# felicityin/zkvm-brainfuck

Hardware: AMD Instinct MI355X
Metric: core-proof wall-time (ms) + NTT HBM GB/s, fibonacci trace 2^22 rows (lower is better)
Workload: dtype u32 (KoalaBear mod-p); 1 GPU; fibo_x4 stdin[255]: 3,767,729 cycles, Cpu trace 2^22 rows, full core proof (84 FRI queries, 16 PoW bits); cycles=3767729, parallelism=replicas x1

## Files before the change

### zkvm-brainfuck_amd/csrc/gpu.h

```cpp
#pragma once
#include <hip/hip_runtime.h>

#include <cstdint>
#include <cstdio>
#include <cstdlib>
#include <functional>
#include <initializer_list>
#include <atomic>
#include <chrono>
#include <map>
#include <mutex>
#include <unordered_map>
#include <unordered_set>
#include <stdexcept>
#include <string>
#include <vector>

#include "kb.h"

namespace bfz {

struct HipError : std::runtime_error {
  using std::runtime_error::runtime_error;
};
// ... 38 lines not shown
      return p;
    }
    if (carve) {
      if (slab_left_ < bytes) {
        if (slab_left_ >= GRAIN) {
          size_of_[slab_next_] = slab_left_;
          free_[slab_left_].push_back(slab_next_);
        }
        slab_next_ = (uint8_t*)device_malloc(SLAB);
        slab_left_ = SLAB;
      }
      void* p = slab_next_;
      slab_next_ += bytes;
      slab_left_ -= bytes;
      size_of_[p] = bytes;
      return p;
    }
    void* p = device_malloc(bytes);
    size_of_[p] = bytes;
    own_.insert(p);
    return p;
  }
  uint64_t mallocs() const { return mallocs_; }
  double malloc_ms() const { return malloc_ns_ * 1e-6; }
  size_t bytes() {
    std::lock_guard<std::mutex> lk(mu_);
    return held_;
  }
  void release(void* p) {
    if (!p) return;
    std::lock_guard<std::mutex> lk(mu_);
    auto it = size_of_.find(p);
    if (it == size_of_.end()) return;
    free_[it->second].push_back(p);
  }
  void trim() {
    std::lock_guard<std::mutex> lk(mu_);
    for (auto kv = free_.begin(); kv != free_.end();) {
      auto& v = kv->second;
      for (size_t i = 0; i < v.size();) {
        if (!own_.count(v[i])) {
          i++;
          continue;
        }
        (void)hipFree(v[i]);
        held_ -= kv->first;
        size_of_.erase(v[i]);
        own_.erase(v[i]);
        v[i] = v.back();
        v.pop_back();
      }
      kv = v.empty() ? free_.erase(kv) : std::next(kv);
    }
  }
  ~DevicePool() {}

 private:
  static bool slabs_on() {
    static const bool on = [] {
      const char* e = std::getenv("BFZ_POOL_SLABS");
      return !(e && e[0] == '0' && !e[1]);
    }();
    return on;
  }
  void* device_malloc(size_t bytes) {
    void* p = nullptr;
    const auto t0 = std::chrono::steady_clock::now();
    HIP_CHECK(hipMalloc(&p, bytes));
    malloc_ns_ += (uint64_t)std::chrono::duration_cast<std::chrono::nanoseconds>(
                      std::chrono::steady_clock::now() - t0).count();
    mallocs_++;
    held_ += bytes;
    return p;
  }
  std::map<size_t, std::vector<void*>> free_;
  std::unordered_map<void*, size_t> size_of_;
  std::unordered_set<void*> own_;
  uint8_t* slab_next_ = nullptr;
  size_t slab_left_ = 0;
  size_t held_ = 0;
  std::atomic<uint64_t> mallocs_{0}, malloc_ns_{0};
  std::mutex mu_;
};

void preload_register(const void* kernel);
struct PreloadKernels {
  PreloadKernels(std::initializer_list<const void*> ks) {
    for (const void* k : ks) preload_register(k);
  }
};
double preload_kernels();

constexpr int MAX_LANES = 4;
constexpr int DEFAULT_INFLIGHT = 2;
struct Lane {
  int id = 0;
  hipStream_t stream = nullptr;
  DevicePool pool;
  uint8_t* stage = nullptr;
  size_t stage_cap = 0, stage_off = 0;
  uint8_t* box = nullptr;
  size_t box_cap = 0;
  hipEvent_t spin = nullptr;
  static constexpr int NGEV = 4;
  hipEvent_t gev[NGEV] = {};
  void* gbox = nullptr;
  size_t gcap = 0;
  uint32_t* tbox = nullptr;
  size_t tcap = 0;
};
Lane& lane();
Lane* lane_at(int i);
size_t lane_pool_bytes(int i);
struct LaneScope {
  Lane* prev;
  explicit LaneScope(Lane* l);
  ~LaneScope();
};

void run_lanes(int n, const std::function<void(int)>& body);

DevicePool& pool();
DevicePool& resident_pool();
struct ResidentScope {
  DevicePool* prev;
  ResidentScope();
  ~ResidentScope();
};

template <class T>
struct DBuf {
  T* p = nullptr;
  size_t n = 0;
  bool owned = true;
  DevicePool* from = nullptr;
  DBuf() = default;
  explicit DBuf(size_t count) { reset(count); }
  DBuf(const DBuf&) = delete;
  DBuf& operator=(const DBuf&) = delete;
  DBuf(DBuf&& o) noexcept : p(o.p), n(o.n), owned(o.owned), from(o.from) { o.p = nullptr; o.n = 0; }
  DBuf& operator=(DBuf&& o) noexcept {
    if (this != &o) { free(); p = o.p; n = o.n; owned = o.owned; from = o.from; o.p = nullptr; o.n = 0; }
    return *this;
  }
  static DBuf borrow(T* ptr, size_t count) {
    DBuf b;
// ... 135 lines not shown
```

### zkvm-brainfuck_amd/csrc/prover.h

```cpp
#pragma once
#include <array>
#include <memory>
#include <string>
#include <vector>

#include "gpu.h"
#include "machine.h"
#include "merkle.h"

namespace bfz {

using kb::EF;

struct Challenger {
  uint32_t st[16] = {0};
  uint32_t in[8] = {0};
  int nin = 0;
  uint32_t out[8] = {0};
  int nout = 0;
  void duplex();
  void observe(uint32_t v);
  void observe_digest(const uint32_t d[8]);
  void observe_ef(const EF& e);
  uint32_t sample();
// ... 50 lines not shown
  double reduce_kernel_ms = 0, reduce_kernel_bytes = 0;
  int reduce_kernel_launches = 0;
  double perm_rows = 0, perm_idft = 0, perm_dft = 0, perm_hash = 0;
  double main_idft = 0, main_dft = 0, main_hash = 0;
  double main_cells = 0, perm_cells = 0;
  double spin = 0;
};

std::unique_ptr<ProvingKey> setup(const std::string& program_src);

void commit_lde(CMat& cm, const uint32_t* evals, size_t n, int w, uint32_t domain_shift,
                hipStream_t st);

struct ProveOptions {
  int num_queries = 84;
  bool timing = false;
  bool observe_openings = true;
  bool fault_device_challenger = false;
};

std::vector<uint8_t> prove(const ProvingKey& pk, const uint8_t* stdin_data, size_t nin,
                           const ProveOptions& opt, StageTimes* times,
                           std::vector<uint8_t>* output_stream = nullptr,
                           uint64_t* cycles = nullptr);

struct DeviceTraces {
  std::vector<int> chips;
  std::vector<DBuf<uint32_t>> evals;
  std::vector<size_t> heights;
};
void upload_host_traces(const int* chips, const uint32_t* const* mats, const size_t* heights,
                        const size_t* widths, size_t n, DeviceTraces& dt, hipStream_t st);
std::vector<uint8_t> prove_device(const ProvingKey& pk, DeviceTraces& dt, const ProveOptions& opt,
                                  StageTimes* times);

void host_mark(const char* what);
std::vector<uint8_t> acquire_proof_buffer();
void release_proof_buffer(std::vector<uint8_t>&& v);

struct MainData {
  DeviceTraces dt;
  std::vector<int> order;
  std::vector<int> chip;
  std::vector<size_t> hn;
  Round mainr;
  bool root_on_host = true;
};
void commit_main(MainData& md);
Challenger challenger_after_pk(const ProvingKey& pk);
std::vector<uint8_t> open_main(const ProvingKey& pk, MainData& md, const Challenger& ch,
                               const ProveOptions& opt, Challenger* after = nullptr);

int num_queries_from_env();
bool observe_openings_from_env();

}
```

### zkvm-brainfuck_amd/csrc/prover.hip

```cpp
#include "prover.h"
#include "pipeline.h"

#include <algorithm>
#include <cerrno>
#include <chrono>
#include <cstdio>
#include <cstdlib>
#include <cstring>
#include <mutex>

#include "fri.h"
#include "host_p2.h"
#include "logup.h"
#include "ntt.h"
#include "poseidon2.h"
#include "quotient.h"
#include "tracegen.h"
#include "verifier.h"

namespace bfz {

using namespace kb;

static constexpr int LOG_BLOWUP = 1;
// ... 325 lines not shown
  if (timed) tm->end(bs, st, split->dft);
  if (tm && tm->on) {
    tm->end(b, st, &times->lde_ms);
    times->lde_bytes += 12.0 * (double)n * w;
    times->lde_elem_stages += 3.0 * (double)n * cm.log_n * w;
    times->lde_calls++;
  }
}

void commit_lde(CMat& cm, const uint32_t* evals, size_t n, int w, uint32_t domain_shift,
                hipStream_t st) {
  lde_into(cm, evals, n, w, domain_shift, st, nullptr, nullptr);
}

static Mailbox* roots_boxes() {
  static Mailbox boxes[MAX_LANES];
  return boxes;
}

static void warm_lane_host() {
  lane_host_reserve();
  Lane& ln = lane();
  roots_boxes()[ln.id].reserve(4096);
  for (int g = 0; g < Lane::NGEV; g++)
    if (!ln.gev[g]) HIP_CHECK(hipEventCreateWithFlags(&ln.gev[g], hipEventDisableTiming));
  if (!ln.gbox) {
    ln.gcap = 4096;
    HIP_CHECK(hipHostMalloc(&ln.gbox, ln.gcap * sizeof(EF), hipHostMallocDefault));
  }
  if (!ln.tbox) {
    ln.tcap = (size_t)1 << 18;
    HIP_CHECK(hipHostMalloc(reinterpret_cast<void**>(&ln.tbox), ln.tcap * 4, hipHostMallocDefault));
  }
}

std::unique_ptr<ProvingKey> setup(const std::string& src) {
  ResidentScope rs;
  warm_lane_host();
  twiddles().ensure(TWIDDLE_LOG_MAX);
  auto pk = std::make_unique<ProvingKey>();
  pk->program = Program::parse(src);
  hipStream_t st = stream();
  int chips[2] = {CHIP_PROGRAM, CHIP_BYTE};
  std::vector<uint32_t> t[2];
  size_t h[2];
  for (int i = 0; i < 2; i++) h[i] = prep_trace(chips[i], pk->program, t[i]);
  int ord[2] = {0, 1};
  if (h[1] > h[0] || (h[1] == h[0] && std::strcmp(CHIP_INFO[chips[1]].name, CHIP_INFO[chips[0]].name) < 0))
    std::swap(ord[0], ord[1]);
  pk->idx_of_chip.fill(-1);
  pk->prep.mats.resize(2);
  pk->prep_evals.resize(2);
  for (int k = 0; k < 2; k++) {
    const int i = ord[k];
    const int w = CHIP_INFO[chips[i]].prep_w;
    pk->chip_of[k] = chips[i];
    pk->idx_of_chip[chips[i]] = k;
    DBuf<uint32_t> rm(h[i] * w);
    HIP_CHECK(hipMemcpyAsync(rm.p, t[i].data(), t[i].size() * 4, hipMemcpyHostToDevice, st));
    pk->prep_evals[k].reset(h[i] * w);
    transpose_bitrev(rm.p, h[i], w, pk->prep_evals[k].p, st);
    HIP_CHECK(hipStreamSynchronize(st));
    lde_into(pk->prep.mats[k], pk->prep_evals[k].p, h[i], w, ONE, st, nullptr, nullptr);
  }
  pk->prep.commit(st);
  return pk;
// ... 1 lines not shown

void upload_host_traces(const int* chips, const uint32_t* const* mats, const size_t* heights,
                        const size_t* widths, size_t n, DeviceTraces& dt, hipStream_t st) {
  dt.chips.clear();
  dt.evals.clear();
  dt.heights.clear();
  bool seen[NUM_CHIPS] = {};
  for (size_t i = 0; i < n; i++) {
    const int c = chips[i];
    if (c < 0 || c >= NUM_CHIPS || seen[c]) throw std::runtime_error("traces: bad or repeated chip id");
    seen[c] = true;
    const size_t h = heights[i];
    const int w = CHIP_INFO[c].main_w;
    if ((size_t)w != widths[i])
      throw std::runtime_error(std::string("traces: width mismatch for ") + CHIP_INFO[c].name);
    if (h < 1 || (h & (h - 1)) || h > ((size_t)1 << 23))
      throw std::runtime_error(std::string("traces: height not a power of two in [1, 2^23] for ") +
                               CHIP_INFO[c].name);
    DBuf<uint32_t> rm(h * w);
    upload_bulk(rm.p, mats[i], h * w * 4, st);
    if (count_noncanonical(rm.p, h * w, st))
      throw std::runtime_error(std::string("traces: non-canonical field word (>= p) in ") +
                               CHIP_INFO[c].name);
    DBuf<uint32_t> ev(h * w);
    transpose_bitrev(rm.p, h, w, ev.p, st);
    dt.chips.push_back(c);
    dt.evals.push_back(std::move(ev));
    dt.heights.push_back(h);
  }
  if (!seen[0]) throw std::runtime_error("traces: the Cpu chip is required");
}

namespace {
struct ProofScope {
  EvTimer ev;
  StageTimes local;
  StageTimes* tms;
  hipEvent_t e_total = nullptr;
  ProofScope(bool timing, StageTimes* times) : tms(times ? times : &local) {
    ev.on = timing && times;
    if (!ev.on) {
      for (KernelProbe* p : {&ntt_probe(), &p2_probe(), &open_probe(), &reduce_probe()})
        if (p->on) p->on = false;
      return;
    }
    ntt_probe().reset();
    ntt_probe().on = true;
    p2_probe().reset();
    p2_probe().on = true;
    open_probe().reset();
    open_probe().on = true;
    reduce_probe().reset();
    reduce_probe().on = true;
    e_total = ev.begin(stream());
  }
  void finish() {
    if (!ev.on) return;
    ev.end(e_total, stream(), &tms->total);
    ev.collect();
    tms->quotient -= tms->spin;
    tms->total -= tms->spin;
    KernelProbe& pr = ntt_probe();
    pr.collect();
    pr.on = false;
    tms->ntt_kernel_ms = pr.ms;
    tms->ntt_kernel_bytes = pr.bytes;
    tms->ntt_kernel_launches = pr.launches;
    KernelProbe& p2 = p2_probe();
    p2.collect();
    p2.on = false;
    tms->p2_kernel_ms = p2.ms;
    tms->p2_perms = p2.bytes;
    tms->p2_launches = p2.launches;
    KernelProbe& op = open_probe();
    op.collect();
    op.on = false;
    tms->open_kernel_ms = op.ms;
    tms->open_kernel_bytes = op.bytes;
    tms->open_kernel_launches = op.launches;
    KernelProbe& rp = reduce_probe();
    rp.collect();
    rp.on = false;
    tms->reduce_kernel_ms = rp.ms;
    tms->reduce_kernel_bytes = rp.bytes;
    tms->reduce_kernel_launches = rp.launches;
  }
  ~ProofScope() {
    (void)hipStreamSynchronize(stream());
    staging_reset();
    if (ev.on)
      for (KernelProbe* p : {&ntt_probe(), &p2_probe(), &open_probe(), &reduce_probe()}) p->on = false;
  }
};

void commit_main_impl(MainData& md, ProofScope& ps, bool fetch_root = true) {
  hipStream_t st = stream();
  DeviceTraces& dt = md.dt;
  const int nc = (int)dt.chips.size();
  md.order.resize(nc);
  for (int i = 0; i < nc; i++) md.order[i] = i;
  std::sort(md.order.begin(), md.order.end(), [&](int a, int b) {
    if (dt.heights[a] != dt.heights[b]) return dt.heights[a] > dt.heights[b];
    return std::strcmp(CHIP_INFO[dt.chips[a]].name, CHIP_INFO[dt.chips[b]].name) < 0;
  });
  md.chip.resize(nc);
  md.hn.resize(nc);
  for (int k = 0; k < nc; k++) {
    md.chip[k] = dt.chips[md.order[k]];
    md.hn[k] = dt.heights[md.order[k]];
  }
  htrace().mark("main commit");
  hipEvent_t e0 = ps.ev.on ? ps.ev.begin(st) : nullptr;
  Span span("commit to main traces");
  const Plan plan = make_plan();
  md.mainr = Round();
  md.mainr.mats.resize(nc);
  LdeSplit split{ps.tms ? &ps.tms->main_idft : nullptr, ps.tms ? &ps.tms->main_dft : nullptr};
  for (int k = 0; k < nc; k++) {
    lde_into(md.mainr.mats[k], dt.evals[md.order[k]].p, md.hn[k], CHIP_INFO[md.chip[k]].main_w, ONE,
             st, &ps.ev, ps.tms, &plan, &chip_next_cols(md.chip[k]).main, ps.tms ? &split : nullptr);
    if (ps.tms) ps.tms->main_cells += (double)md.hn[k] * CHIP_INFO[md.chip[k]].main_w;
  }
  hipEvent_t eh = ps.ev.on ? ps.ev.begin(st) : nullptr;
  htrace().mark("main LDE queued");
  md.mainr.commit(st, fetch_root);
  htrace().mark("main tree queued");
  if (ps.ev.on) ps.ev.end(eh, st, &ps.tms->main_hash);
  md.root_on_host = fetch_root;
  if (ps.ev.on) ps.ev.end(e0, st, &ps.tms->main_commit);
}

std::vector<uint8_t> open_impl(const ProvingKey& pk, MainData& md, Challenger ch,
                               const ProveOptions& opt, ProofScope& ps, Challenger* after = nullptr);

struct QuotXchg {
  std::vector<int> chips;
  std::vector<size_t> off;
  size_t total = 0;
  DBuf<uint32_t> send, recv;
  hipEvent_t ready = nullptr;
  QuotXchg() = default;
  QuotXchg(const QuotXchg&) = delete;
  QuotXchg& operator=(const QuotXchg&) = delete;
  ~QuotXchg() {
    if (ready) (void)hipEventDestroy(ready);
  }
};
static uint32_t* quot_part(std::vector<DBuf<uint32_t>>& qv, const std::vector<size_t>& hn,
                           const Plan& plan, int k, int rank) {
  const size_t n = hn[k], b = plan.blk(2 * n), t0 = (size_t)rank * b;
  return qv[k].p + (t0 / n) * 4 * n + (t0 % n);
}
static void quot_pack(QuotXchg& x, std::vector<DBuf<uint32_t>>& qv, const std::vector<size_t>& hn,
                      const Plan& plan, hipStream_t st) {
  x.off.assign(x.chips.size(), 0);
// ... 35 lines not shown
  for (int j = 0; j < plan.G; j++)
    for (size_t i = 0; i < x.chips.size(); i++)
      if (j != plan.k) {
        const int k = x.chips[i];
        const size_t n = hn[k], b = plan.blk(2 * n);
        cp.push_back({x.recv.p + (size_t)j * x.total + x.off[i], quot_part(qv, hn, plan, k, j), b,
                      n, b, 4});
      }
  copy2d_batch(cp, st);
  x.send.free();
}
}

void commit_main(MainData& md) {
  ProofScope ps(false, nullptr);
  commit_main_impl(md, ps);
  HIP_CHECK(hipStreamSynchronize(stream()));
}

std::vector<uint8_t> open_main(const ProvingKey& pk, MainData& md, const Challenger& ch,
                               const ProveOptions& opt, Challenger* after) {
  ProofScope ps(false, nullptr);
  return open_impl(pk, md, ch, opt, ps, after);
}

Challenger challenger_after_pk(const ProvingKey& pk) {
  Challenger ch;
  ch.observe_digest(pk.prep.tree.root);
  for (int i = 0; i < 7; i++) ch.observe(0);
  return ch;
}

std::vector<uint8_t> prove_device(const ProvingKey& pk, DeviceTraces& dt, const ProveOptions& opt,
                                  StageTimes* times) {
  ProofScope ps(opt.timing, times);
  MainData md;
  md.dt = std::move(dt);
  commit_main_impl(md, ps, false);
  auto proof = open_impl(pk, md, challenger_after_pk(pk), opt, ps);
  htrace().mark("open returned");
  ps.finish();
  dt = std::move(md.dt);
  return proof;
}

namespace {
std::vector<uint8_t> open_impl(const ProvingKey& pk, MainData& md, Challenger ch,
                               const ProveOptions& opt, ProofScope& ps, Challenger* after) {
  hipStream_t st = stream();
  EvTimer& ev = ps.ev;
  StageTimes* tms = ps.tms;
  DeviceTraces& dt = md.dt;
  const std::vector<int>& order = md.order;
  const std::vector<int>& chip = md.chip;
  const std::vector<size_t>& hn = md.hn;
  Round& mainr = md.mainr;
  const int nc = (int)chip.size();
  const Plan plan = make_plan();
  const ShardCtx* shard = shard_ctx();

  htrace().mark("open start");
  DBuf<DevChallenger> dc_d(1);
  {
    DevChallenger dc;
    std::memcpy(dc.st, ch.st, sizeof(dc.st));
    std::memcpy(dc.in, ch.in, sizeof(dc.in));
    std::memcpy(dc.out, ch.out, sizeof(dc.out));
    dc.nin = ch.nin;
    dc.nout = ch.nout;
    if (opt.fault_device_challenger)
      dc.st[15] = dc.st[15] ? dc.st[15] - 1 : 1;
// ... 544 lines not shown
      if (e != hipErrorNotReady) HIP_CHECK(e);
    }
    const size_t b0 = g ? gend[g - 1] : 0, b1 = std::max(gend[g], b0);
    std::copy(gbox + b0, gbox + b1, opened.begin() + b0);
  };
  if (grouped) {
    int have = -1;
    for (int r = 0; r < 4; r++) {
      while (have < group_of(r)) wait_group(++have);
      if (opt.observe_openings)
        for (size_t i = 0; i < rounds[r]->mats.size(); i++)
          for (int j = 0; j < mp[r][i].npts; j++)
            for (int c = 0; c < rounds[r]->mats[i].lde.width; c++)
              ch.observe_ef(opened[mp[r][i].off[j] + c]);
    }
    while (have < NGROUP - 1) wait_group(++have);
    htrace().mark("opened observed");
  } else if (opt.observe_openings) {
    htrace().mark("opened summed");
    for (int r = 0; r < 4; r++)
      for (size_t i = 0; i < rounds[r]->mats.size(); i++)
        for (int j = 0; j < mp[r][i].npts; j++)
          for (int c = 0; c < rounds[r]->mats[i].lde.width; c++)
            ch.observe_ef(opened[mp[r][i].off[j] + c]);
  }
  const EF fri_alpha = ch.sample_ef();
  htrace().mark("fri alpha");

  DBuf<EF> alpha_yab(1 + 2 * std::max<size_t>(red_jobs.size(), 1));
  upload_async(alpha_yab.p, &fri_alpha, sizeof(EF), st);
  reduce_prep(red_cols_d.p, col_prep_d.p, red_mats_d.p, mat_prep_d.p, job_prep_d.p,
              (int)red_jobs.size(), opened_dev, alpha_yab.p, alpha_yab.p + 1, st);
  std::map<int, DBuf<EF>> ro;
  for (size_t ji = 0; ji < red_jobs.size(); ji++) {
    const RedJob& j = red_jobs[ji];
    const size_t H = (size_t)1 << j.lh;
    const bool sh = plan.sharded(H);
    const size_t t0 = sh ? plan.row0(H) : 0, cnt = sh ? plan.blk(H) : H;
    DBuf<EF> r(cnt);
    const Invd& d = invd.at(j.lh);
    reduce_range(red_cols_d.p + j.col0, red_mats_d.p + j.mat0, j.nmats, H, t0, cnt, d.pa(),
                 j.has_b ? d.pb() : nullptr, alpha_yab.p + 1 + 2 * ji, j.has_b, r.p - t0, st,
                 (int)j.ncols);
    ro.emplace(j.lh, std::move(r));
  }
  if (ev.on) ev.end(e3, st, &tms->open);

  hipEvent_t e4 = ev.on ? ev.begin(st) : nullptr;
  struct FriLayer {
    DBuf<EF> v;
    size_t e0 = 0;
    bool local = false;
  };
  std::vector<FriLayer> layers;
  std::vector<MerkleTree> trees;
  {
    const size_t H = (size_t)1 << Lmax;
    layers.push_back({std::move(ro.at(Lmax)), plan.sharded(H) ? plan.row0(H) : 0, plan.sharded(H)});
  }
  ro.erase(Lmax);
  if (ch.nin != 0) throw std::runtime_error("FRI: unexpected pending challenger input");
  DBuf<uint32_t> dstate(16);
  upload_async(dstate.p, ch.st, 64, st);
  const int nrounds = Lmax - LOG_BLOWUP;
  DBuf<EF> betas(std::max(nrounds, 1));
  size_t len = (size_t)1 << Lmax;
  static const size_t FRI_SHARD_MIN = [] {
    const char* e = std::getenv("BFZ_FRI_SHARD_MIN");
    return e ? (size_t)std::strtoull(e, nullptr, 10) : (size_t)1 << 18;
  }();
  auto fri_sharded = [&](size_t h) { return plan.sharded(h) && h >= FRI_SHARD_MIN; };
  auto gather = [&](DBuf<EF>& v, size_t len) {
    DBuf<EF> all(len);
    coll_sync(st);
    shard->allgather(v.p, plan.blk(len) * sizeof(EF), all.p);
    v = std::move(all);
  };
// ... 17 lines not shown
      flush_fold();
      FriTailRounds a;
      a.logh0 = log2i(h);
      a.nr = log2i(len) - LOG_BLOWUP;
      a.in = cur.v.p;
      a.state = dstate.p;
      a.beta = betas.p + rd;
      size_t nw = 0, nv = 0;
      for (int r = 0; r < a.nr; r++) {
        nw += 8 * ((h >> r) * 2 - 1);
        nv += h >> r;
      }
      tail_trees.reset(nw);
      tail_layers.reset(nv);
      nw = nv = 0;
      for (int r = 0; r < a.nr; r++) {
        const size_t hr = h >> r;
        const EF* rows = r ? tail_layers.p + nv - 2 * hr : cur.v.p;
        trees.emplace_back();
        MerkleTree& t = trees.back();
        t.mats = {MatRef{(const uint32_t*)rows, hr, 8}};
        t.layers.resize(log2i(hr) + 1);
        a.tree[r] = tail_trees.p + nw;
        for (size_t L = 0; L < t.layers.size(); L++) {
          t.layers[L] = DBuf<uint32_t>::borrow(tail_trees.p + nw, 8 * (hr >> L));
          nw += 8 * (hr >> L);
        }
        a.layer[r] = tail_layers.p + nv;
        const int lgh = log2i(hr);
        a.add[r] = ro.count(lgh) ? ro.at(lgh).p : nullptr;
        layers.push_back({DBuf<EF>::borrow(tail_layers.p + nv, hr), 0, false});
        nv += hr;
      }
      fri_tail_rounds(a, st);
      len = h >> (a.nr - 1);
      break;
    }
    if (cur.local && !fri_sharded(h)) {
      gather(cur.v, len);
      cur.e0 = 0;
      cur.local = false;
    }
    const bool loc = cur.local;
    const size_t i0 = loc ? plan.row0(h) : 0, cnt = loc ? plan.blk(h) : h;
    trees.emplace_back();
    MerkleTree& t = trees.back();
    std::function<void(size_t, size_t, uint32_t*)> fused;
    if (pend.in) {
      const PendingFold pf = pend;
      EF* out = cur.v.p;
      fused = [pf, out, h, &st](size_t, size_t, uint32_t* dig) {
        fri_fold_leaves(pf.in, out, h, pf.beta, pf.add, dig, st);
      };
      pend = PendingFold{};
    }
    merkle_from_rows8(t, (const uint32_t*)(cur.v.p - 2 * i0), h, st, false,
                      RootChallenge{dstate.p, betas.p + rd}, loc, fused);
    DBuf<EF> next(cnt);
    const int lgh = log2i(h);
    if (!loc && ro.count(lgh) && plan.sharded(h)) gather(ro.at(lgh), h);
    const EF* add = ro.count(lgh) ? ro.at(lgh).p : nullptr;
    if (!loc && h / 2 >= FRI_FUSE_MIN) pend = PendingFold{cur.v.p, betas.p + rd, add, h};
    else fri_fold_range(cur.v.p, next.p, h, i0, cnt, betas.p + rd, add, st);
    layers.push_back({std::move(next), i0, loc});
    len = h;
  }
  flush_fold();
  const int nt = (int)trees.size();
  if (nt > MAX_FRI_ROUNDS) throw std::runtime_error("FRI: too many rounds");
  const int nq = opt.num_queries;

  auto owner_shift = [](const MerkleTree& t, int L) {
    const int nl = (int)t.layers.size() - 1;
    return L < t.sharded_below ? nl - L - t.shard_log : -1;
  };
  std::vector<GatherSeg> segs;
  const int ncommit = nt;
  auto lit = [&](uint32_t v) { segs.push_back({nullptr, 0, 0, v, 0, 1, -1, 0}); };
  lit(4);
  for (int r = 0; r < 4; r++) {
    const Round& R = *rounds[r];
    const int lrm = (int)R.tree.layers.size() - 1;
    lit((uint32_t)R.mats.size());
    for (const CMat& m : R.mats) {
      const int lh = log2i(m.lde.height);
      lit((uint32_t)m.lde.width);
      segs.push_back({m.rows(), (uint64_t)m.stride(), (uint32_t)(Lmax - lh), 0, 1,
                      (uint32_t)m.lde.width, m.sharded ? lh - plan.lg : -1, 0});
    }
    lit((uint32_t)lrm);
    for (int L = 0; L < lrm; L++)
      segs.push_back({R.tree.layers[L].p, 1, (uint32_t)(Lmax - lrm + L), 1, 8, 8,
                      owner_shift(R.tree, L), 0});
  }
  lit((uint32_t)ncommit);
  for (int i = 0; i < ncommit; i++) {
    const FriLayer& fl = layers[i];
    segs.push_back({(const uint32_t*)(fl.v.p - fl.e0), 1, (uint32_t)i, 1, 4, 4,
                    fl.local ? Lmax - i - plan.lg : -1, 0});
    const int lm = (int)trees[i].layers.size() - 1;
// ... 112 lines not shown
    write_vals(mp[2][k].off[1], pw);
    w.u32(2);
    write_vals(mp[3][2 * k].off[0], 4);
    write_vals(mp[3][2 * k + 1].off[0], 4);
    w.ef(cums[k]);
  }
  w.u32((uint32_t)ncommit);
  for (int i = 0; i < ncommit; i++) w.digest(trees[i].root);
  w.u32((uint32_t)nq);
  w.raw(words, nwords);
  w.ef(fin[0]);
  w.u32(witness);
  htrace().mark("serialized");
  return w.take();
}
}

std::vector<uint8_t> prove_events(const ProvingKey& pk, const DeviceEvents& ev,
                                  const ProveOptions& opt, StageTimes* times) {
  hipStream_t st = stream();
  const bool timing = opt.timing && times;
  hipEvent_t a = nullptr, b = nullptr;
  if (timing) {
    HIP_CHECK(hipEventCreate(&a));
    HIP_CHECK(hipEventCreate(&b));
    HIP_CHECK(hipEventRecord(a, st));
  }
  htrace().mark("proof start", true);
  static const bool pool_diag = std::getenv("BFZ_HOST_TRACE") != nullptr;
  const uint64_t m0 = lane().pool.mallocs();
  const double t0 = lane().pool.malloc_ms();
  Span span("prove_shard");
  DeviceTraces dt;
  {
    Span gen("generate traces for shard");
    generate_traces_device(ev, dt, st);
  }
  htrace().mark("traces launched");
  if (timing) HIP_CHECK(hipEventRecord(b, st));
  auto proof = prove_device(pk, dt, opt, times);
  htrace().mark("proof returned");
  if (pool_diag)
    std::fprintf(stderr, "pool: %llu hipMalloc in this proof, %.3f ms of host time\n",
                 (unsigned long long)(lane().pool.mallocs() - m0), lane().pool.malloc_ms() - t0);
  if (timing) {
    float ms = 0;
    HIP_CHECK(hipEventElapsedTime(&ms, a, b));
    times->trace = ms;
    times->total += ms;
    HIP_CHECK(hipEventDestroy(a));
    HIP_CHECK(hipEventDestroy(b));
  }
  return proof;
}

std::vector<uint8_t> prove(const ProvingKey& pk, const uint8_t* in, size_t nin,
                           const ProveOptions& opt, StageTimes* times,
                           std::vector<uint8_t>* output_stream, uint64_t* cycles) {
  HostEvents& h = scratch_events();
  execute_into(pk.program, in, nin, h);
  DeviceEvents ev;
  upload_events(h, pk.program, ev, stream());
  if (output_stream) *output_stream = h.output;
  if (cycles) *cycles = h.global_clk;
  return prove_events(pk, ev, opt, times);
}

static PreloadKernels preload_prover{(const void*)&k_pack_fri_tail};

}
```

### zkvm-brainfuck_amd/csrc/runtime.hip

```cpp
#include <dlfcn.h>

#include "gpu.h"

#include <algorithm>
#include <condition_variable>
#include <cstring>
#include <mutex>
#include <thread>
#include <vector>

namespace bfz {

namespace {
std::mutex g_lanes_mu;
Lane* g_lanes[MAX_LANES] = {};
thread_local Lane* tl_lane = nullptr;
Lane* make_lane(int id) {
  auto* l = new Lane();
  l->id = id;
  HIP_CHECK(hipStreamCreateWithFlags(&l->stream, hipStreamNonBlocking));
  return l;
}
}

Lane* lane_at(int i) {
  if (i < 0 || i >= MAX_LANES) throw std::runtime_error("lane index out of range");
  std::lock_guard<std::mutex> lk(g_lanes_mu);
  if (!g_lanes[i]) g_lanes[i] = make_lane(i);
  return g_lanes[i];
}
size_t lane_pool_bytes(int i) {
  if (i < 0 || i >= MAX_LANES) throw std::runtime_error("lane index out of range");
  Lane* l;
  {
    std::lock_guard<std::mutex> lk(g_lanes_mu);
    l = g_lanes[i];
  }
  return l ? l->pool.bytes() : 0;
}
Lane& lane() {
  if (tl_lane) return *tl_lane;
  static Lane* d = lane_at(0);
  return *d;
}
LaneScope::LaneScope(Lane* l) : prev(tl_lane) { tl_lane = l; }
LaneScope::~LaneScope() { tl_lane = prev; }

namespace {
thread_local DevicePool* tl_pool = nullptr;
}
DevicePool& pool() { return tl_pool ? *tl_pool : lane().pool; }
DevicePool& resident_pool() {
  static DevicePool* p = new DevicePool();
// ... 13 lines not shown
  std::call_once(once, [&] {
    const char* e = std::getenv("BFZ_PRELOAD");
    if (e && e[0] == '0' && !e[1]) return;
    const auto t0 = std::chrono::steady_clock::now();
    for (const void* k : preload_list()) {
      hipFuncAttributes a;
      HIP_CHECK(hipFuncGetAttributes(&a, k));
    }
    ms = std::chrono::duration<double, std::milli>(std::chrono::steady_clock::now() - t0).count();
  });
  return ms;
}

void run_lanes(int n, const std::function<void(int)>& body) {
  std::exception_ptr err;
  std::mutex mu;
  auto one = [&](int i) {
    try {
      ApiLockScope held;
      LaneScope ls(lane_at(i));
      body(i);
      HIP_CHECK(hipStreamSynchronize(stream()));
    } catch (...) {
      std::lock_guard<std::mutex> lk(mu);
      if (!err) err = std::current_exception();
    }
  };
  std::vector<std::thread> th;
  for (int i = 1; i < n; i++) th.emplace_back(one, i);
  one(0);
  for (auto& t : th) t.join();
  if (err) std::rethrow_exception(err);
}
hipStream_t stream() { return lane().stream; }

void quiesce() noexcept {
  for (Lane* l : g_lanes)
    if (l && l->stream) (void)hipStreamSynchronize(l->stream);
}

namespace {
struct Roctx {
  int (*push)(const char*) = nullptr;
  int (*pop)() = nullptr;
  Roctx() {
    void* h = dlopen("librocprofiler-sdk-roctx.so", RTLD_NOW | RTLD_LOCAL);
    if (!h) h = dlopen("/opt/rocm/lib/librocprofiler-sdk-roctx.so", RTLD_NOW | RTLD_LOCAL);
    if (!h) return;
    push = reinterpret_cast<int (*)(const char*)>(dlsym(h, "roctxRangePushA"));
    pop = reinterpret_cast<int (*)()>(dlsym(h, "roctxRangePop"));
    if (!push || !pop) push = nullptr, pop = nullptr;
  }
};
const Roctx& roctx() {
  static const Roctx r;
  return r;
}
}
void roctx_push(const char* name) noexcept {
  if (roctx().push) roctx().push(name);
}
void roctx_pop() noexcept {
  if (roctx().pop) roctx().pop();
}

KernelProbe& ntt_probe() {
  static KernelProbe* k = new KernelProbe();
  return *k;
}

KernelProbe& p2_probe() {
// ... 333 lines not shown
```

### zkvm-brainfuck_amd/csrc/tracegen.h

```cpp
#pragma once
#include "gpu.h"
#include "machine.h"
#include "prover.h"

namespace bfz {

struct DeviceEvents {
  DBuf<CpuEvent> cpu;
  DBuf<AluEvent> alu;
  DBuf<JumpEvent> jump;
  DBuf<MemInstrEvent> meminstr;
  DBuf<IoEvent> io;
  DBuf<MemoryEvent> memory;
  DBuf<Instruction> prog;
  size_t n[NUM_CHIPS] = {};
  size_t height[NUM_CHIPS] = {};
  bool included[NUM_CHIPS] = {};
  uint64_t global_clk = 0;
};

void upload_events(const ExecutionRecord& rec, DeviceEvents& ev, hipStream_t st);

void upload_events(const HostEvents& h, const Program& prog, DeviceEvents& ev, hipStream_t st);
void set_event_meta(DeviceEvents& ev, const EventCounts& n, uint64_t global_clk);
size_t count_invalid_events(const DeviceEvents& ev, hipStream_t st);
void expand_cycles(const Cycle* d, size_t n, DeviceEvents& ev, EventCounts& n_out, size_t* invalid,
                   hipStream_t st);
void* pinned_alloc(size_t bytes);
void pinned_free(void* p);

void generate_traces_device(const DeviceEvents& ev, DeviceTraces& dt, hipStream_t st);

std::vector<uint8_t> prove_events(const ProvingKey& pk, const DeviceEvents& ev,
                                  const ProveOptions& opt, StageTimes* times);

}
```

### zkvm-brainfuck_amd/csrc/tracegen.hip

```cpp
#include "tracegen.h"
#include "ntt.h"
#include "quotient.h"

namespace bfz {

using namespace kb;

namespace {

__device__ __forceinline__ uint32_t mb(bool b) { return b ? ONE : 0u; }

__device__ __forceinline__ void put_word(uint32_t* c, uint32_t v) {
#pragma unroll
  for (int i = 0; i < 4; i++) c[i] = to_mont((v >> (8 * i)) & 0xff);
}

__device__ __forceinline__ void put_word_rc(uint32_t* c, uint32_t v) {
  uint32_t b[8];
#pragma unroll
  for (int i = 0; i < 8; i++) b[i] = (v >> (i + 24)) & 1;
#pragma unroll
  for (int i = 0; i < 8; i++) c[i] = mb(b[i]);
  uint32_t a = b[0] & b[1];
  c[8] = mb(a);
// ... 536 lines not shown
                     (const Instruction*)ev.prog.p, nprog, bc.p, cnt.p);
  KCHECK();
  hipLaunchKernelGGL(k_cycles_scan, dim3(1), dim3(1024), 0, st, bc.p, nb, cnt.p);
  KCHECK();
  uint32_t h[NCAT + 1];
  fetch(h, cnt.p, sizeof h, st);
  *invalid = h[NCAT];
  n_out.cpu = n;
  n_out.alu = h[CAT_ALU];
  n_out.jump = h[CAT_JUMP];
  n_out.meminstr = h[CAT_MEM];
  n_out.io = h[CAT_IO];
  ev.cpu.reset(n);
  ev.alu.reset(std::max<size_t>(n_out.alu, 1));
  ev.jump.reset(std::max<size_t>(n_out.jump, 1));
  ev.meminstr.reset(std::max<size_t>(n_out.meminstr, 1));
  ev.io.reset(std::max<size_t>(n_out.io, 1));
  if (*invalid) return;
  hipLaunchKernelGGL(k_cycles_expand, dim3((unsigned)nb), dim3(XB), 0, st, d, n,
                     (const Instruction*)ev.prog.p, nprog, (const uint32_t*)bc.p, ev.cpu.p, ev.alu.p,
                     ev.jump.p, ev.meminstr.p, ev.io.p);
  KCHECK();
}

void* pinned_alloc(size_t bytes) {
  void* p = nullptr;
  if (hipHostMalloc(&p, bytes, hipHostMallocDefault) != hipSuccess) return nullptr;
  return p;
}
void pinned_free(void* p) {
  if (p) (void)hipHostFree(p);
}

void generate_traces_device(const DeviceEvents& ev, DeviceTraces& dt, hipStream_t st) {
  dt.chips.clear();
  dt.evals.clear();
  dt.heights.clear();
  if (ev.n[CHIP_CPU] > 0xffffffffull / 4) throw std::runtime_error("tracegen: too many cycles");
  const int nprog = (int)ev.n[CHIP_PROGRAM];
  DBuf<uint32_t> m8(256), m16(65536), mprog(std::max(nprog, 1));
  HIP_CHECK(hipMemsetAsync(m8.p, 0, 256 * 4, st));
  HIP_CHECK(hipMemsetAsync(m16.p, 0, 65536 * 4, st));
  HIP_CHECK(hipMemsetAsync(mprog.p, 0, std::max(nprog, 1) * 4, st));
  {
    const size_t work = std::max(ev.n[CHIP_CPU], ev.n[CHIP_ADDSUB]);
    const unsigned grid = std::max(1u, std::min<unsigned>(ceil_div(work, 256 * 16), 1024));
    hipLaunchKernelGGL(k_deps, dim3(grid), dim3(256), 0, st, (const CpuEvent*)ev.cpu.p,
                       ev.n[CHIP_CPU], (const AluEvent*)ev.alu.p, ev.n[CHIP_ADDSUB], m8.p, m16.p,
                       mprog.p, nprog);
    KCHECK();
  }
  for (int c = 0; c < NUM_CHIPS; c++) {
    if (!ev.included[c]) continue;
    const size_t h = ev.height[c];
    const int w = CHIP_INFO[c].main_w;
    const int logh = log2i(h);
    DBuf<uint32_t> out(h * (size_t)w);
    const dim3 grid(ceil_div(h, 256)), blk(256);
    switch (c) {
      case CHIP_CPU:
        hipLaunchKernelGGL(k_trace_cpu, grid, blk, 0, st, (const CpuEvent*)ev.cpu.p, ev.n[c],
                           (const Instruction*)ev.prog.p, out.p, h, logh);
        break;
      case CHIP_PROGRAM:
        hipLaunchKernelGGL(k_trace_program, grid, blk, 0, st, (const uint32_t*)mprog.p, ev.n[c],
                           out.p, h, logh);
        break;
      case CHIP_ADDSUB:
        hipLaunchKernelGGL(k_trace_addsub, grid, blk, 0, st, (const AluEvent*)ev.alu.p, ev.n[c],
                           out.p, h, logh);
        break;
      case CHIP_JUMP:
        hipLaunchKernelGGL(k_trace_jump, grid, blk, 0, st, (const JumpEvent*)ev.jump.p, ev.n[c],
                           out.p, h, logh);
        break;
      case CHIP_MEMORY:
        hipLaunchKernelGGL(k_trace_memory, grid, blk, 0, st, (const MemoryEvent*)ev.memory.p,
                           ev.n[c], out.p, h, logh);
        break;
      case CHIP_BYTE:
        hipLaunchKernelGGL(k_trace_byte, grid, blk, 0, st, (const uint32_t*)m8.p,
                           (const uint32_t*)m16.p, out.p);
        break;
      case CHIP_MEMINSTRS:
        hipLaunchKernelGGL(k_trace_meminstr, grid, blk, 0, st, (const MemInstrEvent*)ev.meminstr.p,
                           ev.n[c], out.p, h, logh);
        break;
      case CHIP_IO:
        hipLaunchKernelGGL(k_trace_io, grid, blk, 0, st, (const IoEvent*)ev.io.p, ev.n[c], out.p, h,
                           logh);
        break;
    }
    KCHECK();
    dt.chips.push_back(c);
    dt.evals.push_back(std::move(out));
    dt.heights.push_back(h);
  }
}

static PreloadKernels preload_tracegen{
    (const void*)&k_deps,
    (const void*)&k_trace_cpu,
    (const void*)&k_trace_addsub,
    (const void*)&k_trace_jump,
    (const void*)&k_trace_memory,
    (const void*)&k_trace_meminstr,
    (const void*)&k_trace_io,
    (const void*)&k_trace_program,
    (const void*)&k_trace_byte};

}
```

Baseline: 27.17 ms.

## Overlap non-CPU trace generation and FRI reduce jobs on a side stream

Adds a per-lane side stream with fork/join events and a SideScope helper. The CPU trace is generated on the main stream, while the other chips' traces and the dependency counting run on the side stream. The main LDE waits on the side stream only before it needs a non-CPU chip. FRI reduce jobs after the first also run on the side stream and are joined before the fold that consumes them. Pool releases made during side sections are parked until the join, so buffers are not reused across streams. This adds event-sync complexity and may cause contention between the concurrent kernels.

After: 27.12 ms, median of 3. No clear change (-0.2%).

```diff
diff --git a/zkvm-brainfuck_amd/csrc/gpu.h b/zkvm-brainfuck_amd/csrc/gpu.h
--- a/zkvm-brainfuck_amd/csrc/gpu.h
+++ b/zkvm-brainfuck_amd/csrc/gpu.h
@@ -94,7 +94,15 @@
     std::lock_guard<std::mutex> lk(mu_);
     auto it = size_of_.find(p);
     if (it == size_of_.end()) return;
+    if (sink_) {
+      sink_->push_back(p);
+      return;
+    }
     free_[it->second].push_back(p);
+  }
+  void defer_to(std::vector<void*>* sink) {
+    std::lock_guard<std::mutex> lk(mu_);
+    sink_ = sink;
   }
   void trim() {
     std::lock_guard<std::mutex> lk(mu_);
@@ -141,6 +149,7 @@
   uint8_t* slab_next_ = nullptr;
   size_t slab_left_ = 0;
   size_t held_ = 0;
+  std::vector<void*>* sink_ = nullptr;
   std::atomic<uint64_t> mallocs_{0}, malloc_ns_{0};
   std::mutex mu_;
 };
@@ -158,6 +167,10 @@
 struct Lane {
   int id = 0;
   hipStream_t stream = nullptr;
+  hipStream_t side = nullptr;
+  static constexpr int NSIDE = 2;
+  hipEvent_t side_ev[2 * NSIDE] = {};
+  bool on_side = false;
   DevicePool pool;
   uint8_t* stage = nullptr;
   size_t stage_cap = 0, stage_off = 0;
@@ -174,6 +187,21 @@
 Lane& lane();
 Lane* lane_at(int i);
 size_t lane_pool_bytes(int i);
+struct SideScope {
+  Lane& ln;
+  const bool on;
+  const int site;
+  bool in = false, marked = false, joined = false;
+  std::vector<void*> parked;
+  SideScope(bool on, int site);
+  SideScope(const SideScope&) = delete;
+  SideScope& operator=(const SideScope&) = delete;
+  void fork();
+  hipStream_t enter();
+  void leave();
+  void join();
+  ~SideScope();
+};
 struct LaneScope {
   Lane* prev;
   explicit LaneScope(Lane* l);
diff --git a/zkvm-brainfuck_amd/csrc/prover.h b/zkvm-brainfuck_amd/csrc/prover.h
--- a/zkvm-brainfuck_amd/csrc/prover.h
+++ b/zkvm-brainfuck_amd/csrc/prover.h
@@ -106,7 +106,7 @@
 void upload_host_traces(const int* chips, const uint32_t* const* mats, const size_t* heights,
                         const size_t* widths, size_t n, DeviceTraces& dt, hipStream_t st);
 std::vector<uint8_t> prove_device(const ProvingKey& pk, DeviceTraces& dt, const ProveOptions& opt,
-                                  StageTimes* times);
+                                  StageTimes* times, SideScope* traces = nullptr);
 
 void host_mark(const char* what);
 std::vector<uint8_t> acquire_proof_buffer();
diff --git a/zkvm-brainfuck_amd/csrc/prover.hip b/zkvm-brainfuck_amd/csrc/prover.hip
--- a/zkvm-brainfuck_amd/csrc/prover.hip
+++ b/zkvm-brainfuck_amd/csrc/prover.hip
@@ -381,6 +381,15 @@
     ln.tcap = (size_t)1 << 18;
     HIP_CHECK(hipHostMalloc(reinterpret_cast<void**>(&ln.tbox), ln.tcap * 4, hipHostMallocDefault));
   }
+  for (int site = 0; site < Lane::NSIDE; site++) {
+    DBuf<uint32_t> scratch(64);
+    SideScope warm(true, site);
+    hipStream_t ss = warm.enter();
+    HIP_CHECK(hipMemsetAsync(scratch.p, 0, 64 * sizeof(uint32_t), ss));
+    warm.leave();
+    warm.join();
+    HIP_CHECK(hipStreamSynchronize(ln.stream));
+  }
 }
 
 std::unique_ptr<ProvingKey> setup(const std::string& src) {
@@ -448,13 +457,33 @@
 }
 
 namespace {
+enum SideSite {
+  SIDE_TRACES = 0,
+  SIDE_REDUCE = 1,
+};
+static_assert(SIDE_REDUCE < Lane::NSIDE, "lane side events");
+struct SideCfg {
+  unsigned mask = 0;
+  bool site(int s) const { return (mask >> s) & 1; }
+};
+SideCfg side_config(bool timed) {
+  SideCfg c;
+  const ShardCtx* sh = shard_ctx();
+  if (timed || (sh && sh->world > 1)) return c;
+  c.mask = (1u << Lane::NSIDE) - 1;
+  if (const char* e = std::getenv("BFZ_SIDE")) c.mask &= (unsigned)std::strtoul(e, nullptr, 0);
+  return c;
+}
+
 struct ProofScope {
   EvTimer ev;
   StageTimes local;
   StageTimes* tms;
   hipEvent_t e_total = nullptr;
+  SideCfg side;
   ProofScope(bool timing, StageTimes* times) : tms(times ? times : &local) {
     ev.on = timing && times;
+    side = side_config(ev.on);
     if (!ev.on) {
       for (KernelProbe* p : {&ntt_probe(), &p2_probe(), &open_probe(), &reduce_probe()})
         if (p->on) p->on = false;
@@ -509,7 +538,8 @@
   }
 };
 
-void commit_main_impl(MainData& md, ProofScope& ps, bool fetch_root = true) {
+void commit_main_impl(MainData& md, ProofScope& ps, bool fetch_root = true,
+                      SideScope* traces = nullptr) {
   hipStream_t st = stream();
   DeviceTraces& dt = md.dt;
   const int nc = (int)dt.chips.size();
@@ -533,10 +563,12 @@
   md.mainr.mats.resize(nc);
   LdeSplit split{ps.tms ? &ps.tms->main_idft : nullptr, ps.tms ? &ps.tms->main_dft : nullptr};
   for (int k = 0; k < nc; k++) {
+    if (traces && md.chip[k] != CHIP_CPU) traces->join();
     lde_into(md.mainr.mats[k], dt.evals[md.order[k]].p, md.hn[k], CHIP_INFO[md.chip[k]].main_w, ONE,
              st, &ps.ev, ps.tms, &plan, &chip_next_cols(md.chip[k]).main, ps.tms ? &split : nullptr);
     if (ps.tms) ps.tms->main_cells += (double)md.hn[k] * CHIP_INFO[md.chip[k]].main_w;
   }
+  if (traces) traces->join();
   hipEvent_t eh = ps.ev.on ? ps.ev.begin(st) : nullptr;
   htrace().mark("main LDE queued");
   md.mainr.commit(st, fetch_root);
@@ -638,11 +670,11 @@
 }
 
 std::vector<uint8_t> prove_device(const ProvingKey& pk, DeviceTraces& dt, const ProveOptions& opt,
-                                  StageTimes* times) {
+                                  StageTimes* times, SideScope* traces) {
   ProofScope ps(opt.timing, times);
   MainData md;
   md.dt = std::move(dt);
-  commit_main_impl(md, ps, false);
+  commit_main_impl(md, ps, false, traces);
   auto proof = open_impl(pk, md, challenger_after_pk(pk), opt, ps);
   htrace().mark("open returned");
   ps.finish();
@@ -1253,17 +1285,32 @@
   reduce_prep(red_cols_d.p, col_prep_d.p, red_mats_d.p, mat_prep_d.p, job_prep_d.p,
               (int)red_jobs.size(), opened_dev, alpha_yab.p, alpha_yab.p + 1, st);
   std::map<int, DBuf<EF>> ro;
-  for (size_t ji = 0; ji < red_jobs.size(); ji++) {
-    const RedJob& j = red_jobs[ji];
+  auto job_range = [&](const RedJob& j, size_t& t0, size_t& cnt) {
     const size_t H = (size_t)1 << j.lh;
     const bool sh = plan.sharded(H);
-    const size_t t0 = sh ? plan.row0(H) : 0, cnt = sh ? plan.blk(H) : H;
-    DBuf<EF> r(cnt);
+    t0 = sh ? plan.row0(H) : 0;
+    cnt = sh ? plan.blk(H) : H;
+  };
+  for (const RedJob& j : red_jobs) {
+    size_t t0, cnt;
+    job_range(j, t0, cnt);
+    ro.emplace(j.lh, DBuf<EF>(cnt));
+  }
+  auto reduce_job = [&](size_t ji, hipStream_t st) {
+    const RedJob& j = red_jobs[ji];
+    size_t t0, cnt;
+    job_range(j, t0, cnt);
     const Invd& d = invd.at(j.lh);
-    reduce_range(red_cols_d.p + j.col0, red_mats_d.p + j.mat0, j.nmats, H, t0, cnt, d.pa(),
-                 j.has_b ? d.pb() : nullptr, alpha_yab.p + 1 + 2 * ji, j.has_b, r.p - t0, st,
-                 (int)j.ncols);
-    ro.emplace(j.lh, std::move(r));
+    reduce_range(red_cols_d.p + j.col0, red_mats_d.p + j.mat0, j.nmats, (size_t)1 << j.lh, t0, cnt,
+                 d.pa(), j.has_b ? d.pb() : nullptr, alpha_yab.p + 1 + 2 * ji, j.has_b,
+                 ro.at(j.lh).p - t0, st, (int)j.ncols);
+  };
+  if (!red_jobs.empty()) reduce_job(0, st);
+  SideScope rside(ps.side.site(SIDE_REDUCE) && red_jobs.size() > 1, SIDE_REDUCE);
+  {
+    hipStream_t ss = rside.enter();
+    for (size_t ji = 1; ji < red_jobs.size(); ji++) reduce_job(ji, ss);
+    rside.leave();
   }
   if (ev.on) ev.end(e3, st, &tms->open);
 
@@ -1347,6 +1394,7 @@
         layers.push_back({DBuf<EF>::borrow(tail_layers.p + nv, hr), 0, false});
         nv += hr;
       }
+      rside.join();
       fri_tail_rounds(a, st);
       len = h >> (a.nr - 1);
       break;
@@ -1374,6 +1422,7 @@
     DBuf<EF> next(cnt);
     const int lgh = log2i(h);
     if (!loc && ro.count(lgh) && plan.sharded(h)) gather(ro.at(lgh), h);
+    if (ro.count(lgh)) rside.join();
     const EF* add = ro.count(lgh) ? ro.at(lgh).p : nullptr;
     if (!loc && h / 2 >= FRI_FUSE_MIN) pend = PendingFold{cur.v.p, betas.p + rd, add, h};
     else fri_fold_range(cur.v.p, next.p, h, i0, cnt, betas.p + rd, add, st);
@@ -1381,6 +1430,7 @@
     len = h;
   }
   flush_fold();
+  rside.join();
   const int nt = (int)trees.size();
   if (nt > MAX_FRI_ROUNDS) throw std::runtime_error("FRI: too many rounds");
   const int nq = opt.num_queries;
@@ -1559,13 +1609,15 @@
   const double t0 = lane().pool.malloc_ms();
   Span span("prove_shard");
   DeviceTraces dt;
+  SideScope tside(side_config(timing).site(SIDE_TRACES), SIDE_TRACES);
   {
     Span gen("generate traces for shard");
-    generate_traces_device(ev, dt, st);
-  }
+    generate_traces_device(ev, dt, st, &tside);
+  }
+
   htrace().mark("traces launched");
   if (timing) HIP_CHECK(hipEventRecord(b, st));
-  auto proof = prove_device(pk, dt, opt, times);
+  auto proof = prove_device(pk, dt, opt, times, &tside);
   htrace().mark("proof returned");
   if (pool_diag)
     std::fprintf(stderr, "pool: %llu hipMalloc in this proof, %.3f ms of host time\n",
diff --git a/zkvm-brainfuck_amd/csrc/runtime.hip b/zkvm-brainfuck_amd/csrc/runtime.hip
--- a/zkvm-brainfuck_amd/csrc/runtime.hip
+++ b/zkvm-brainfuck_amd/csrc/runtime.hip
@@ -19,6 +19,8 @@
   auto* l = new Lane();
   l->id = id;
   HIP_CHECK(hipStreamCreateWithFlags(&l->stream, hipStreamNonBlocking));
+  HIP_CHECK(hipStreamCreateWithFlags(&l->side, hipStreamNonBlocking));
+  for (hipEvent_t& e : l->side_ev) HIP_CHECK(hipEventCreateWithFlags(&e, hipEventDisableTiming));
   return l;
 }
 }
@@ -98,11 +100,66 @@
   for (auto& t : th) t.join();
   if (err) std::rethrow_exception(err);
 }
-hipStream_t stream() { return lane().stream; }
+hipStream_t stream() {
+  Lane& l = lane();
+  return l.on_side ? l.side : l.stream;
+}
 
 void quiesce() noexcept {
-  for (Lane* l : g_lanes)
+  for (Lane* l : g_lanes) {
+    if (l && l->side) (void)hipStreamSynchronize(l->side);
     if (l && l->stream) (void)hipStreamSynchronize(l->stream);
+  }
+}
+
+SideScope::SideScope(bool enable, int s) : ln(lane()), on(enable), site(s) {
+  if (!on) return;
+  if (site < 0 || site >= Lane::NSIDE) throw std::logic_error("SideScope: bad site");
+  fork();
+}
+void SideScope::fork() {
+  if (!on) return;
+  if (in || marked) throw std::logic_error("SideScope: fork after the section");
+  HIP_CHECK(hipEventRecord(ln.side_ev[2 * site], ln.stream));
+}
+hipStream_t SideScope::enter() {
+  if (!on) return ln.stream;
+  if (in || marked || ln.on_side) throw std::logic_error("SideScope: section opened twice");
+  in = true;
+  ln.on_side = true;
+  ln.pool.defer_to(&parked);
+  HIP_CHECK(hipStreamWaitEvent(ln.side, ln.side_ev[2 * site], 0));
+  return ln.side;
+}
+void SideScope::leave() {
+  if (!in) return;
+  in = false;
+  ln.on_side = false;
+  ln.pool.defer_to(nullptr);
+  marked = true;
+  HIP_CHECK(hipEventRecord(ln.side_ev[2 * site + 1], ln.side));
+}
+void SideScope::join() {
+  if (!on || joined) return;
+  leave();
+  joined = true;
+  if (!marked) HIP_CHECK(hipEventRecord(ln.side_ev[2 * site + 1], ln.side));
+  HIP_CHECK(hipStreamWaitEvent(ln.stream, ln.side_ev[2 * site + 1], 0));
+  for (void* p : parked) ln.pool.release(p);
+  parked.clear();
+}
+SideScope::~SideScope() {
+  if (!on || joined) return;
+  try {
+    join();
+  } catch (...) {
+    in = false;
+    ln.on_side = false;
+    ln.pool.defer_to(nullptr);
+    (void)hipStreamSynchronize(ln.side);
+    for (void* p : parked) ln.pool.release(p);
+    parked.clear();
+  }
 }
 
 namespace {
diff --git a/zkvm-brainfuck_amd/csrc/tracegen.h b/zkvm-brainfuck_amd/csrc/tracegen.h
--- a/zkvm-brainfuck_amd/csrc/tracegen.h
+++ b/zkvm-brainfuck_amd/csrc/tracegen.h
@@ -29,7 +29,8 @@
 void* pinned_alloc(size_t bytes);
 void pinned_free(void* p);
 
-void generate_traces_device(const DeviceEvents& ev, DeviceTraces& dt, hipStream_t st);
+void generate_traces_device(const DeviceEvents& ev, DeviceTraces& dt, hipStream_t st,
+                            SideScope* side = nullptr);
 
 std::vector<uint8_t> prove_events(const ProvingKey& pk, const DeviceEvents& ev,
                                   const ProveOptions& opt, StageTimes* times);
diff --git a/zkvm-brainfuck_amd/csrc/tracegen.hip b/zkvm-brainfuck_amd/csrc/tracegen.hip
--- a/zkvm-brainfuck_amd/csrc/tracegen.hip
+++ b/zkvm-brainfuck_amd/csrc/tracegen.hip
@@ -592,12 +592,23 @@
   if (p) (void)hipHostFree(p);
 }
 
-void generate_traces_device(const DeviceEvents& ev, DeviceTraces& dt, hipStream_t st) {
+static void generate_chip(const DeviceEvents& ev, int c, const uint32_t* m8, const uint32_t* m16,
+                          const uint32_t* mprog, DeviceTraces& dt, hipStream_t st);
+
+void generate_traces_device(const DeviceEvents& ev, DeviceTraces& dt, hipStream_t main_st,
+                            SideScope* side) {
   dt.chips.clear();
   dt.evals.clear();
   dt.heights.clear();
   if (ev.n[CHIP_CPU] > 0xffffffffull / 4) throw std::runtime_error("tracegen: too many cycles");
   const int nprog = (int)ev.n[CHIP_PROGRAM];
+  const bool split = side && side->on;
+  hipStream_t st = main_st;
+  if (split) {
+    if (ev.included[CHIP_CPU]) generate_chip(ev, CHIP_CPU, nullptr, nullptr, nullptr, dt, main_st);
+    side->fork();
+    st = side->enter();
+  }
   DBuf<uint32_t> m8(256), m16(65536), mprog(std::max(nprog, 1));
   HIP_CHECK(hipMemsetAsync(m8.p, 0, 256 * 4, st));
   HIP_CHECK(hipMemsetAsync(m16.p, 0, 65536 * 4, st));
@@ -610,52 +621,59 @@
                        mprog.p, nprog);
     KCHECK();
   }
-  for (int c = 0; c < NUM_CHIPS; c++) {
-    if (!ev.included[c]) continue;
-    const size_t h = ev.height[c];
-    const int w = CHIP_INFO[c].main_w;
-    const int logh = log2i(h);
-    DBuf<uint32_t> out(h * (size_t)w);
-    const dim3 grid(ceil_div(h, 256)), blk(256);
-    switch (c) {
-      case CHIP_CPU:
-        hipLaunchKernelGGL(k_trace_cpu, grid, blk, 0, st, (const CpuEvent*)ev.cpu.p, ev.n[c],
-                           (const Instruction*)ev.prog.p, out.p, h, logh);
-        break;
-      case CHIP_PROGRAM:
-        hipLaunchKernelGGL(k_trace_program, grid, blk, 0, st, (const uint32_t*)mprog.p, ev.n[c],
-                           out.p, h, logh);
-        break;
-      case CHIP_ADDSUB:
-        hipLaunchKernelGGL(k_trace_addsub, grid, blk, 0, st, (const AluEvent*)ev.alu.p, ev.n[c],
-                           out.p, h, logh);
-        break;
-      case CHIP_JUMP:
-        hipLaunchKernelGGL(k_trace_jump, grid, blk, 0, st, (const JumpEvent*)ev.jump.p, ev.n[c],
-                           out.p, h, logh);
-        break;
-      case CHIP_MEMORY:
-        hipLaunchKernelGGL(k_trace_memory, grid, blk, 0, st, (const MemoryEvent*)ev.memory.p,
-                           ev.n[c], out.p, h, logh);
-        break;
-      case CHIP_BYTE:
-        hipLaunchKernelGGL(k_trace_byte, grid, blk, 0, st, (const uint32_t*)m8.p,
-                           (const uint32_t*)m16.p, out.p);
-        break;
-      case CHIP_MEMINSTRS:
-        hipLaunchKernelGGL(k_trace_meminstr, grid, blk, 0, st, (const MemInstrEvent*)ev.meminstr.p,
-                           ev.n[c], out.p, h, logh);
-        break;
-      case CHIP_IO:
-        hipLaunchKernelGGL(k_trace_io, grid, blk, 0, st, (const IoEvent*)ev.io.p, ev.n[c], out.p, h,
-                           logh);
-        break;
-    }
-    KCHECK();
-    dt.chips.push_back(c);
-    dt.evals.push_back(std::move(out));
-    dt.heights.push_back(h);
-  }
+  for (int c = split ? CHIP_CPU + 1 : 0; c < NUM_CHIPS; c++)
+    if (ev.included[c]) generate_chip(ev, c, m8.p, m16.p, mprog.p, dt, st);
+  if (split) {
+    m8.free();
+    m16.free();
+    mprog.free();
+    side->leave();
+  }
+}
+
+static void generate_chip(const DeviceEvents& ev, int c, const uint32_t* m8, const uint32_t* m16,
+                          const uint32_t* mprog, DeviceTraces& dt, hipStream_t st) {
+  const size_t h = ev.height[c];
+  const int w = CHIP_INFO[c].main_w;
+  const int logh = log2i(h);
+  DBuf<uint32_t> out(h * (size_t)w);
+  const dim3 grid(ceil_div(h, 256)), blk(256);
+  switch (c) {
+    case CHIP_CPU:
+      hipLaunchKernelGGL(k_trace_cpu, grid, blk, 0, st, (const CpuEvent*)ev.cpu.p, ev.n[c],
+                         (const Instruction*)ev.prog.p, out.p, h, logh);
+      break;
+    case CHIP_PROGRAM:
+      hipLaunchKernelGGL(k_trace_program, grid, blk, 0, st, mprog, ev.n[c], out.p, h, logh);
+      break;
+    case CHIP_ADDSUB:
+      hipLaunchKernelGGL(k_trace_addsub, grid, blk, 0, st, (const AluEvent*)ev.alu.p, ev.n[c],
+                         out.p, h, logh);
+      break;
+    case CHIP_JUMP:
+      hipLaunchKernelGGL(k_trace_jump, grid, blk, 0, st, (const JumpEvent*)ev.jump.p, ev.n[c],
+                         out.p, h, logh);
+      break;
+    case CHIP_MEMORY:
+      hipLaunchKernelGGL(k_trace_memory, grid, blk, 0, st, (const MemoryEvent*)ev.memory.p,
+                         ev.n[c], out.p, h, logh);
+      break;
+    case CHIP_BYTE:
+      hipLaunchKernelGGL(k_trace_byte, grid, blk, 0, st, m8, m16, out.p);
+      break;
+    case CHIP_MEMINSTRS:
+      hipLaunchKernelGGL(k_trace_meminstr, grid, blk, 0, st, (const MemInstrEvent*)ev.meminstr.p,
+                         ev.n[c], out.p, h, logh);
+      break;
+    case CHIP_IO:
+      hipLaunchKernelGGL(k_trace_io, grid, blk, 0, st, (const IoEvent*)ev.io.p, ev.n[c], out.p, h,
+                         logh);
+      break;
+  }
+  KCHECK();
+  dt.chips.push_back(c);
+  dt.evals.push_back(std::move(out));
+  dt.heights.push_back(h);
 }
 
 static PreloadKernels preload_tracegen{
```
